# jviquerat/beacon

Hardware: AMD Instinct MI355X
Metric: aggregate env steps/sec, rayleigh-v0 batch=512/GPU 128x64 (higher is better)
Workload: dtype f32

## Files before the change

### beacon_amd/build.py

```python
import fcntl
import glob
import hashlib
import os
import shutil
import subprocess
from concurrent.futures import ThreadPoolExecutor

PKG = os.path.dirname(os.path.abspath(__file__))
CSRC = os.path.join(PKG, "csrc")
INC = os.path.join(os.path.dirname(PKG), "include")
LIB = os.path.join(PKG, "libbeacon_hip.so")
OBJ = os.path.join(PKG, "csrc", "_obj")
ARCH = "gfx950"
FLAGS = ["-O3", "-std=c++17", "-fPIC", "--offload-arch=" + ARCH, "-fvisibility=hidden",
         "-fgpu-rdc" if False else "-fno-gpu-rdc", "-Wall", "-Wno-unused-function",
         "-Wno-unused-variable", "-Wno-unused-but-set-variable"]


FILE_FLAGS = {"ns2d_fast.hip": ["-fno-slp-vectorize", "-ffp-contract=on", "-O2"],
              "ns2d_fast_f64.hip": ["-fno-slp-vectorize", "-ffp-contract=on"],
              "ns2d_fast2.hip": ["-fno-slp-vectorize", "-ffp-contract=on", "-mllvm", "-amdgpu-disable-unclustered-high-rp-reschedule",
                                 "-mllvm", "-amdgpu-sdwa-peephole=0"],
              "ns2d_fast_prm.hip": ["-fno-slp-vectorize", "-ffp-contract=on", "-O2"],
              "ns2d_fast_prm_f64.hip": ["-fno-slp-vectorize", "-ffp-contract=on"],
              "ns2d_fast2_prm.hip": ["-fno-slp-vectorize", "-ffp-contract=on", "-mllvm", "-amdgpu-disable-unclustered-high-rp-reschedule",
                                     "-mllvm", "-amdgpu-sdwa-peephole=0"],
              "env1d_f64.hip": ["-ffp-contract=off"],
              "shkadov_warm_f64.hip": ["-ffp-contract=off"],
              "ode_f64.hip": ["-ffp-contract=off"]}


JIT_FLAGS = ["-fno-slp-vectorize", "-ffp-contract=on"]


def hipcc():
    for c in (os.environ.get("HIPCC"), shutil.which("hipcc"), "/opt/rocm/bin/hipcc"):
        if c and os.path.exists(c):
            return c
    return None


def sources():
    return sorted(glob.glob(os.path.join(CSRC, "*.hip")))


def _deps():
    return (sources() + glob.glob(os.path.join(CSRC, "*.h")) + glob.glob(os.path.join(CSRC, "*.inc")) +
            glob.glob(os.path.join(INC, "*.h")))


def signature():
    h = hashlib.sha256()
    h.update(repr((ARCH, FLAGS, sorted(FILE_FLAGS.items()))).encode())
    for f in sorted(_deps()):
        h.update(os.path.basename(f).encode())
        with open(f, "rb") as fh:
            h.update(fh.read())
    return h.hexdigest()


def stale():
    if not os.path.exists(LIB) or not os.path.exists(LIB + ".sig"):
        return True
    with open(LIB + ".sig") as fh:
        return fh.read().strip() != signature()


def sweep_objdirs():
    if not os.path.isdir(OBJ):
        return
    for d in os.listdir(OBJ):
        if not (d.startswith("p") and d[1:].isdigit()):
            continue
        pid = int(d[1:])
        if pid != os.getpid():
            try:
                os.kill(pid, 0)
                continue
            except ProcessLookupError:
                pass
            except OSError:
                continue
        shutil.rmtree(os.path.join(OBJ, d), ignore_errors=True)


def build_lib(force=False, verbose=False):
    if not force and not stale():
        sweep_objdirs()
        return LIB
    cc = hipcc()
    if cc is None:
        raise RuntimeError("hipcc not found: cannot build libbeacon_hip.so")
    os.makedirs(OBJ, exist_ok=True)
    with open(os.path.join(OBJ, ".lock"), "w") as lock:
        fcntl.flock(lock, fcntl.LOCK_EX)
        try:
            if not force and not stale():
                return LIB
            sig = signature()
            objdir = os.path.join(OBJ, "p%d" % os.getpid())
            os.makedirs(objdir, exist_ok=True)

# ... 29 lines not shown
```

### beacon_amd/csrc/capi.hip

```cpp
#include <math.h>
#include <stdarg.h>
#include <stddef.h>

#include <new>
#include <vector>

#include "env1d.h"
#include "ns2d.h"
#include "ode_env.h"
#include "params.h"
#include "snapshot.h"
#include "episode.h"
#include "shkadov_jets.h"
#include "normalize.h"

static thread_local char g_err[512] = "";

__attribute__((visibility("default"))) void bcn_set_error(const char* fmt, ...) {
  va_list ap;
  va_start(ap, fmt);
  vsnprintf(g_err, sizeof(g_err), fmt, ap);
  va_end(ap);
}

// ... 148 lines not shown
  size_t state_elems() const override { return 4 * (size_t)a.ncell; }
  int get_state(void* buf, int is_device, hipStream_t s) override {
    return copy_planes(buf, fields.p, 4, (size_t)a.ncell * sizeof(real), batch, is_device, s, true);
  }
  int set_state(const void* buf, int is_device, hipStream_t s) override {
    return copy_planes(const_cast<void*>(buf), fields.p, 4, (size_t)a.ncell * sizeof(real), batch, is_device, s, false);
  }
  int set_variant(int v) override { variant = (v == 1 && fast_ok) ? 1 : 0; host.launched = nullptr; return variant; }
  void set_mask(const uint8_t* m) override { a.mask = m; }
  int set_sched(int mode, int grid, int q, int lpt_min_batch) override {
    a.sched_mode = mode; a.sched_grid = grid; a.sched_q_user = q; a.lpt_min_batch = lpt_min_batch;
    return BCN_OK;
  }
  int set_option(const char* name, int value) override {
    if (!strcmp(name, "conv_plan") && value >= 0 && value <= 3) {
      if (value >= 2 && !guard_holds()) { bcn_set_error("conv_plan %d needs a grid with no side below 48 cells (%dx%d): plans 0, 1 only", value, a.nx, a.ny); return BCN_ERR_ARG; }
      a.conv_plan = value;
      return BCN_OK;
    }
    if (!strcmp(name, "plan_overshoot") && value >= 0 && value <= 64) { a.plan_overshoot = value; return BCN_OK; }
    if (!strcmp(name, "verify_conv")) { a.verify_conv = value ? 1 : 0; return BCN_OK; }
    if (!strcmp(name, "spec_start") && value >= 0 && value <= 17) { a.spec_start = value; return BCN_OK; }
    if (!strcmp(name, "transport_iter") && value >= 0 && value <= 64) { a.transport_iter = value; return BCN_OK; }
    if (!strcmp(name, "sched_tail") && value >= 0 && value <= 1024) { host.sched_tail = value; return BCN_OK; }
    if (!strcmp(name, "generic_threads") && (value == 0 || value == 256 || value == 1024)) { host.generic_nt = value; return BCN_OK; }
    if (!strcmp(name, "params_kernel") && (value == 0 || value == 1)) { params_kernel = value; host.launched = nullptr; return BCN_OK; }
    return bcn_env_s::set_option(name, value);
  }
  int get_counters(uint64_t* host, hipStream_t s) override {
    BCN_HIP(hipMemcpyAsync(host, a.cyc, (size_t)batch * 4 * sizeof(uint64_t), hipMemcpyDeviceToHost, s));
    BCN_HIP(hipStreamSynchronize(s));
    return BCN_OK;
  }
  typedef int (*plugin_fn)(const void*, int, void*);
  plugin_fn plugin = nullptr;
  int set_fast_plugin(void* fn, size_t scratch_elems) override {
    plugin_prm = nullptr;
    if (!fn) { plugin = nullptr; fast_ok = ns2d_fast_supported<real>(a); variant = fast_ok ? 1 : 0; return BCN_OK; }
    if (scratch_elems > 0) {
      DeviceGuard g(device);
      fscrbuf.release();
      int rc = fscrbuf.alloc((size_t)batch * scratch_elems * sizeof(real));
      if (rc) return rc;
      BCN_HIP(hipMemset(fscrbuf.p, 0, fscrbuf.bytes));
      a.fscr = static_cast<real*>(fscrbuf.p);
      a.fscr_stride = scratch_elems;
    }
    plugin = reinterpret_cast<plugin_fn>(fn);
    fast_ok = true; variant = 1; host.launched = nullptr;
    return BCN_OK;
  }
  typedef int (*plugin_prm_fn)(const void*, int, void*, const void*);
  plugin_prm_fn plugin_prm = nullptr;
  int set_fast_plugin_params(void* fn) override {
    if (fn && !plugin) { bcn_set_error("bcn_set_fast_plugin_params: the handle has no kernel plugin (bcn_set_fast_plugin comes first)"); return BCN_ERR_ARG; }
    plugin_prm = reinterpret_cast<plugin_prm_fn>(fn);
    host.launched = nullptr;
    return BCN_OK;
  }
  NS2DHost host;
  const real* prm = nullptr;
  int params_kernel = 0;
  void use_params(const void* table) override { prm = static_cast<const real*>(table); host.launched = nullptr; }
  bool prm_fast() const {
    return prm && params_kernel == 1 && variant == 1 && (plugin ? plugin_prm != nullptr : ns2d_fast_supported_prm<real>(a));
  }
  const char* kernel_name() const override {
    if (prm && !prm_fast()) return "ns2d_generic_step";
    return host.launched ? host.launched : (variant == 1 ? "ns2d_fast_step" : "ns2d_generic_step");
  }
  int launch(hipStream_t s) {
    a.host = &host;
    if (prm) {
      if (prm_fast()) {
        const int rc = plugin ? plugin_prm(&a, batch, s, prm) : ns2d_launch_fast_prm<real>(a, batch, s, prm);
        if (rc != BCN_ERR_UNSUPPORTED) return rc;
      }
      return ns2d_launch_generic_prm<real>(a, batch, s, prm);
    }
    if (variant == 1 && plugin) {
      const int rc = plugin(&a, batch, s);
      if (rc != BCN_ERR_UNSUPPORTED) return rc;
      return ns2d_launch_generic<real>(a, batch, s);
    }
    if (variant == 1) return ns2d_launch_fast<real>(a, batch, s);
    return ns2d_launch_generic<real>(a, batch, s);
  }
};

template <typename real>
void ns2d_common(NS2DArgs<real>& a, int nx, int ny, double dx, double dy, double dt, double tol) {
  a.nx = nx; a.ny = ny; a.sx = nx + 2; a.ncell = (nx + 2) * (ny + 2);
  a.dt = (real)dt; a.rdx = (real)(1.0 / dx); a.rdy = (real)(1.0 / dy);
  a.rdx2 = (real)(1.0 / (dx * dx)); a.rdy2 = (real)(1.0 / (dy * dy));
  const double den = dx * dx + dy * dy;
  a.cx = (real)(0.5 * dy * dy / den);
  a.cy = (real)(0.5 * dx * dx / den);
  a.cb = (real)(0.5 * dx * dx * dy * dy / den / dt);
  a.tol = (real)tol;
}

template <typename real>
int make_rayleigh(const bcn_rayleigh_cfg* c, int batch, int dtype, int device, bcn_env_t* out) {
  return make_env<NS2DEnv<real>>(BCN_RAYLEIGH, batch, dtype, device, snap_cfg_hash<bcn_rayleigh_cfg, 12, 9>(c), out, [c](NS2DEnv<real>* e) {
    NS2DArgs<real>& a = e->a;
    ns2d_common(a, c->nx, c->ny, c->dx, c->dy, c->dt, c->tol);
    a.kind = 0; a.ndt_act = c->ndt_act; a.n_act = c->n_act; a.itmax = c->itmax;
    a.n_sgts = c->n_sgts; a.nx_sgts = c->nx_sgts;
    a.nxo = c->nx_obs_pts; a.nyo = c->ny_obs_pts; a.nx_obs = c->nx_obs; a.ny_obs = c->ny_obs;
    a.n_obs_steps = c->n_obs_steps; a.n_obs = 3 * c->n_obs_steps * c->nx_obs_pts * c->ny_obs_pts;
    a.kmom = (real)bcn_rayleigh_kmom(c->pr, c->ra);
    a.ksc = (real)bcn_rayleigh_ksc(c->pr, c->ra);
    e->prm_cfg[0] = c->ra; e->prm_aux[0] = c->pr;
    a.Tc = (real)c->Tc; a.Th = (real)c->Th; a.C = (real)c->C;
    a.rwd_scale = (real)(1.0 / (0.5 * c->dy * c->nx));
    e->n_obs = a.n_obs; e->n_act = c->n_sgts; e->ndt_act = a.ndt_act;
  });
}

template <typename real>
int make_mixing(const bcn_mixing_cfg* c, int batch, int dtype, int device, bcn_env_t* out) {
  return make_env<NS2DEnv<real>>(BCN_MIXING, batch, dtype, device, snap_cfg_hash<bcn_mixing_cfg, 14, 9>(c), out, [c](NS2DEnv<real>* e) {
    NS2DArgs<real>& a = e->a;
    ns2d_common(a, c->nx, c->ny, c->dx, c->dy, c->dt, c->tol);
    a.kind = 1; a.ndt_act = c->ndt_act; a.n_act = c->n_act; a.itmax = c->itmax;
    a.n_sgts = 0; a.nx_sgts = 1;
    a.nxo = c->nx_obs_pts; a.nyo = c->ny_obs_pts; a.nx_obs = c->nx_obs; a.ny_obs = c->ny_obs;
    a.n_obs_steps = c->n_obs_steps; a.n_obs = 3 * c->n_obs_steps * c->nx_obs_pts * c->ny_obs_pts;
    a.i_min = c->i_min; a.i_max = c->i_max; a.j_min = c->j_min; a.j_max = c->j_max;
    a.kmom = (real)bcn_mixing_kmom(c->re);
    a.ksc = (real)bcn_mixing_ksc(c->pe);
    e->prm_cfg[0] = c->re; e->prm_cfg[1] = c->pe; e->prm_aux[0] = c->re; e->prm_aux[1] = c->u_max;
    a.u_max = (real)bcn_mixing_u_max(c->re, c->re, c->u_max); a.ref_c = (real)c->ref_c; a.C0 = (real)c->C0;
    e->n_obs = a.n_obs; e->n_act = 1; e->ndt_act = a.ndt_act;
  });
}

template <typename real>
struct Env1D : bcn_env_s {
  Env1DArgs<real> a{};
  int nfields = 4;
  int nact = 1;
  DevBuf fields, a_last, a_prev, stpbuf, nctrbuf;
  const char* general = "";
  Env1DLaunch last;

  int init() {
    int rc;
    const size_t per = (size_t)batch * a.n * sizeof(real);
    if ((rc = fields.alloc(4 * per))) return rc;
    BCN_HIP(hipMemset(fields.p, 0, 4 * per));
    real* f = static_cast<real*>(fields.p);
    const size_t n = (size_t)batch * a.n;
    a.f0 = f; a.f1 = f + n; a.f2 = f + 2 * n; a.f3 = f + 3 * n;
    if ((rc = a_last.alloc((size_t)batch * nact * sizeof(real)))) return rc;
    if ((rc = a_prev.alloc((size_t)batch * nact * sizeof(real)))) return rc;
    BCN_HIP(hipMemset(a_last.p, 0, a_last.bytes));
    BCN_HIP(hipMemset(a_prev.p, 0, a_prev.bytes));
    a.a_last = static_cast<real*>(a_last.p);
    a.a_prev = static_cast<real*>(a_prev.p);
    if ((rc = stpbuf.alloc((size_t)batch * sizeof(int32_t)))) return rc;
    BCN_HIP(hipMemset(stpbuf.p, 0, stpbuf.bytes));
    stp = a.stp = static_cast<int32_t*>(stpbuf.p);
    if ((rc = nctrbuf.alloc((size_t)batch * sizeof(uint32_t)))) return rc;
    BCN_HIP(hipMemset(nctrbuf.p, 0, nctrbuf.bytes));
    a.nctr = static_cast<uint32_t*>(nctrbuf.p);
// ... 941 lines not shown
```

### beacon_amd/csrc/ns2d.h

```cpp
#pragma once
#include "bcn_common.h"

struct NS2DHost {
  const char* launched = nullptr;
  int sched_tail = 0;
  int generic_nt = 0;
};

template <typename real>
struct NS2DArgs {
  int nx, ny, sx, ncell;
  int ndt_act, n_act, itmax;
  int kind;
  int n_sgts, nx_sgts;
  int nxo, nyo, nx_obs, ny_obs, n_obs_steps, n_obs;
  int i_min, i_max, j_min, j_max;
  real dt, rdx, rdy, rdx2, rdy2;
  real kmom;
  real ksc;
  real cx, cy, cb;
  real tol;
  real Tc, Th, C, u_max, ref_c, C0;
  real rwd_scale;
  real *u, *v, *p, *S, *us, *vs;
  real *g0, *g1, *g2;
  real* obs_hist;
  real* a_last;
  int32_t* ia_last;
  int32_t* stp;
  const real* actions;
  const int32_t* iactions;
  real* actions_norm;
  real* obs_out;
  real* rwd_out;
  uint8_t* done;
  uint8_t* trunc;
  int32_t* status;
  int32_t* sweeps;
  const real* init_fields;
  const uint8_t* mask;
  int work_in_lds;
  int it_begin, it_end;
  int first_chunk, last_chunk;
  const int32_t* order;
  int32_t* order_out;
  int32_t* sweeps_int;
  void* sched_ctl;
  unsigned long long* cyc;
  size_t sched_bytes;
  int sched_q;
  int sched_nbig = 0;
  int conv_plan = 1;
  int plan_overshoot = 0;
  int spec_start = 0;
  int verify_conv = 0;
  int sched_mode = -1;
  int sched_grid = 0, sched_q_user = 0, lpt_min_batch = 0;
  NS2DHost* host;
  real* fscr;
  size_t fscr_stride;
  int transport_iter = 0;
  float slow_l2lc[2] = {0.f, 0.f};
  float slow_cl[2] = {__builtin_inff(), __builtin_inff()};
};

template <typename real> int ns2d_launch_generic(const NS2DArgs<real>& a, int batch, hipStream_t s);
template <typename real> int ns2d_launch_reset(const NS2DArgs<real>& a, int batch, hipStream_t s);
size_t ns2d_generic_lds_bytes(int ncell, size_t esz);
template <typename real> bool ns2d_fast_supported(const NS2DArgs<real>& a);
template <typename real> int ns2d_launch_fast(const NS2DArgs<real>& a, int batch, hipStream_t s);
template <typename real> size_t ns2d_fast_scratch_elems(const NS2DArgs<real>& a);
template <typename real> bool ns2d_fast2_supported(const NS2DArgs<real>& a);
template <typename real> size_t ns2d_fast2_scratch_elems(const NS2DArgs<real>& a);
template <typename real> int ns2d_launch_fast2(const NS2DArgs<real>& a, int batch, hipStream_t s);
```

### beacon_amd/csrc/ns2d_fast.hip

```cpp
#include "ns2d_fast_impl.h"

namespace {

template <typename real>
int fast_config(const NS2DArgs<real>& a) {
  if (a.kind != 0 || a.n_sgts > 64) return 0;
  if (a.nx == 128 && a.ny == 64 && sizeof(real) == 4) return 1;
  if (a.nx == 50 && a.ny == 50) return 2;
  if (a.nx == 128 && a.ny == 64 && sizeof(real) == 8) return 3;
  if (a.nx == 100 && a.ny == 50 && sizeof(real) == 4) return 4;
  if (a.nx == 150 && a.ny == 50 && sizeof(real) == 4) return 5;
  if (a.nx == 200 && a.ny == 50 && sizeof(real) == 4) return 6;
  return 0;
}

}

template <typename real>
bool BCN_PRM_NAME(ns2d_fast_supported)(const NS2DArgs<real>& a) { return fast_config<real>(a) != 0 || BCN_PRM_NAME(ns2d_fast2_supported)<real>(a); }

template <typename real>
int BCN_PRM_NAME(ns2d_launch_fast)(const NS2DArgs<real>& a, int batch, hipStream_t s BCN_PRM_PARAM) {
  if (BCN_PRM_NAME(ns2d_fast2_supported)<real>(a)) return BCN_PRM_NAME(ns2d_launch_fast2)<real>(a, batch, s BCN_PRM_ARG);
  switch (fast_config<real>(a)) {
    case 1:
      if constexpr (std::is_same<real, float>::value) return launch_fast<float, 128, 64, BCN_R128, 0>(a, batch, s BCN_PRM_ARG);
      break;
    case 2: return launch_fast<real, 50, 50, BCN_R50, 0>(a, batch, s BCN_PRM_ARG);
    case 3:
      if constexpr (std::is_same<real, double>::value) return launch_fast<double, 128, 64, BCN_R128D, 0, BCN_GFD>(a, batch, s BCN_PRM_ARG);
      break;
    case 4:
      if constexpr (std::is_same<real, float>::value) return launch_fast<float, 100, 50, 10, 0>(a, batch, s BCN_PRM_ARG);
      break;
    case 5:
      if constexpr (std::is_same<real, float>::value) return launch_fast<float, 150, 50, 15, 0>(a, batch, s BCN_PRM_ARG);
      break;
    case 6:
      if constexpr (std::is_same<real, float>::value) return launch_fast<float, 200, 50, 25, 0>(a, batch, s BCN_PRM_ARG);
      break;
    default: break;
  }
  bcn_set_error("no register-resident kernel for this grid");
  return BCN_ERR_UNSUPPORTED;
}

#ifndef BCN_PRM_KERNELS
template <typename real>
size_t ns2d_fast_scratch_elems(const NS2DArgs<real>& a) {
  if (ns2d_fast2_supported<real>(a)) return ns2d_fast2_scratch_elems<real>(a);
  if (fast_config<real>(a) == 3) return FastGeom<128, 64, BCN_R128D, BCN_GFD>::scratch_elems();
  return 0;
}
#endif
#ifdef BCN_PRM_KERNELS
#ifndef BCN_FAST_TU_F64
template bool ns2d_fast_supported_prm<float>(const NS2DArgs<float>&);
template int ns2d_launch_fast_prm<float>(const NS2DArgs<float>&, int, hipStream_t, const float*);
#else
template bool ns2d_fast_supported_prm<double>(const NS2DArgs<double>&);
template int ns2d_launch_fast_prm<double>(const NS2DArgs<double>&, int, hipStream_t, const double*);
#endif
#elif !defined(BCN_FAST_TU_F64)
template size_t ns2d_fast_scratch_elems<float>(const NS2DArgs<float>&);
template bool ns2d_fast_supported<float>(const NS2DArgs<float>&);
template int ns2d_launch_fast<float>(const NS2DArgs<float>&, int, hipStream_t);
#else
template size_t ns2d_fast_scratch_elems<double>(const NS2DArgs<double>&);
template bool ns2d_fast_supported<double>(const NS2DArgs<double>&);
template int ns2d_launch_fast<double>(const NS2DArgs<double>&, int, hipStream_t);
#endif
```

### beacon_amd/csrc/ns2d_fast_impl.h

```cpp
#pragma once
#include <stdlib.h>

#include <type_traits>

#include "bcn_dpp.h"
#include "ns2d.h"
#include "ns2d_device.h"
#include "ns2d_prm.h"
#include "ns2d_sched.h"


#ifndef BCN_R128
#define BCN_R128 16
#endif
#ifndef BCN_R50
#define BCN_R50 5
#endif
#ifndef BCN_GFD
#define BCN_GFD 2
#endif
#ifndef BCN_PDG
#define BCN_PDG 8
#endif
static_assert(BCN_PDG == 4 || BCN_PDG == 8 || BCN_PDG == 10 || BCN_PDG == 12 || BCN_PDG == 16 || BCN_PDG == 20,
// ... 177 lines not shown
    }                                                                                       \
  }
  constexpr int TA = ((NY - 1 + PD - 1) / PD) * PD;
  constexpr int TB = (NX / PD) * PD;
  if constexpr (TA <= TB) {
    BCN_CHAIN(0, TA, 1)
    if (NY == 64) { BCN_CHAIN(TA, TB, 0) } else { BCN_CHAIN(TA, TB, 1) }
    BCN_CHAIN(TB, NSTEP, 2)
  } else {
    constexpr int TL = ((NY - 1) / PD) * PD, TH = ((NX + PD - 1) / PD) * PD;
    BCN_CHAIN(0, TL, 1)
    BCN_CHAIN(TL, TH, 3)
    BCN_CHAIN(TH, NSTEP, 2)
  }
#undef BCN_CHAIN
}

template <typename real, int NX, int NY, int R0, int RW, int KIND, bool EQ, int GF>
__device__ __forceinline__ void fast_body(const NS2DArgs<real>& A, const int w, const int b, const int it_begin, const int it_end,
                                          const bool first_chunk, const bool last_chunk, char* smem) {
  using G = FastGeom<NX, NY, R0, GF>;
  constexpr int R = RW;
  constexpr int NW = G::NW, NT = G::NT, SY = G::SY, SX = G::SX, SZ = G::SZ, PD = G::PD;
  real* exch = reinterpret_cast<real*>(smem);
  real* errp = exch + G::EXCH;
  real* sact = errp + 128;
  real* red = sact + 64;
  real* gscr = GF ? A.fscr + (size_t)blockIdx.x * A.fscr_stride + G::FRONTG : nullptr;
  real* Ul = GF == 1 ? gscr : GF == 2 ? exch + G::MISCA : exch + G::FRONT;
  real* Vl = Ul + SZ;
  real* Tl = GF == 2 ? gscr : Vl + SZ;

  const int tid = threadIdx.x, lane = tid & 63;
  int j = lane + 1;
  const bool active = lane < NY;
  constexpr int RL = G::RL;
  constexpr bool DEADC = GF == 2 && RW == R0 && RL != R0;
  static_assert(!(DEADC && G::XC == 4), "dead columns exist only in the single-sweep exchange paths (XC == 2, GF == 2)");
  const bool lastw = DEADC && w == NW - 1;
#define LIVE(k) (!DEADC || (k) < RL || !lastw)
  const int i0 = w * R0 + 1;
  const size_t off = (size_t)b * A.ncell;
  real* __restrict__ gu = A.u + off;
  real* __restrict__ gv = A.v + off;
  real* __restrict__ gp = A.p + off;
  real* __restrict__ gS = A.S + off;
  constexpr int XC = G::XC, XL = XC - 1;
  auto exl = [&](int buf, int wave, int which) -> real& { return exch[((buf * NW + wave) * XC + which) * 64 + lane]; };

  for (int c = tid; c < SX * SY; c += NT) {
    const int jj = c / SX, ii = c - jj * SX;
    Ul[ii * SY + jj] = gu[c];
    Vl[ii * SY + jj] = gv[c];
    Tl[ii * SY + jj] = gS[c];
  }
  for (int c = SX * SY + tid; c < SZ; c += NT) { Ul[c] = 0; Vl[c] = 0; Tl[c] = 0; }
  if (tid < 128) errp[tid] = 0;
  real p[R];
#pragma unroll
  for (int k = 0; k < R; k++) p[k] = (active && LIVE(k)) ? gp[j * SX + i0 + k] : real(0);

  if (!first_chunk) {
    if (tid < A.n_sgts) sact[tid] = A.a_last[(size_t)b * A.n_sgts + tid];
  } else {
    const int n = A.n_sgts;
    const real* src = A.actions ? A.actions + (size_t)b * n : A.a_last + (size_t)b * n;
    real mean = 0;
    for (int k = 0; k < n; k++) mean += src[k];
    mean /= (real)n;
    real m = 1;
    for (int k = 0; k < n; k++) {
      real t = bcn_abs(src[k] - mean) / A.C;
      m = t > m ? t : m;
    }
    real mine = (tid < n) ? (src[tid] - mean) / m : real(0);
    __syncthreads();
    if (tid < n) {
      sact[tid] = mine;
      A.a_last[(size_t)b * n + tid] = mine;
      if (A.actions_norm) A.actions_norm[(size_t)b * n + tid] = mine;
    }
  }
  __syncthreads();

  const real dt = A.dt, rdx = A.rdx, rdy = A.rdy, rdx2 = A.rdx2, rdy2 = A.rdy2;
  const real cx = A.cx, cy = A.cy;
  const real wl = active ? real(1) + (j == 1 ? 1 : 0) + ((j == NY && KIND == 0) ? 1 : 0) : real(0);
  const real fW = (active && w == 0) ? real(1) : real(0);
  const real fE = (active && w == NW - 1) ? real(1) : real(0);
  const real cW = wl + fW, cE = lastw ? real(0) : wl + fE;
  const real fEl = lastw ? fE : real(0);
  const real cBy = cy * (real)((lane == 0 ? 1 : 0) + ((lane == NY - 1 && KIND == 0) ? 1 : 0));
  const real actf = active ? real(1) : real(0);

  int status = 0;
  int xb = 0;
#ifdef BCN_STAMP
  const unsigned long long kt0 = __builtin_amdgcn_s_memtime(), kr0 = __builtin_amdgcn_s_memrealtime();
  unsigned long long seg[7] = {0, 0, 0, 0, 0, 0, 0};
  unsigned long long tl = kt0;
#define BCN_PH(x) { __builtin_amdgcn_sched_barrier(0); const unsigned long long t__ = __builtin_amdgcn_s_memtime(); seg[x] += t__ - tl; tl = t__; __builtin_amdgcn_sched_barrier(0); }
#else
#define BCN_PH(x)
#endif
  if (!first_chunk) status = A.status[b];
  const unsigned long long cyc_u0 = __builtin_amdgcn_s_memtime();
  unsigned long long cyc_j = 0;
  real* const prev_sweeps = red + 20;
  constexpr bool SPEC = std::is_same<real, float>::value;
#if !defined(BCN_STAMP) && !defined(BCN_DBG_NCHK)
  if (tid == 0) prev_sweeps[0] = (it_begin > 0 && A.sweeps) ? (real)A.sweeps[(size_t)b * A.ndt_act + it_begin - 1] : real(0);
#else
  if (tid == 0) prev_sweeps[0] = 0;
#endif
  if (tid == 0) { prev_sweeps[1] = 0; prev_sweeps[2] = 0; prev_sweeps[3] = 0; }
  real* const slow_k = red + 24;
  if (tid == 0) {
    slow_k[0] = 0; slow_k[5] = 0;
    slow_k[1] = (real)A.slow_l2lc[0]; slow_k[2] = (real)A.slow_cl[0];
    slow_k[3] = (real)A.slow_l2lc[1]; slow_k[4] = (real)A.slow_cl[1];
  }

  constexpr bool OFFLOAD = G::template offload<real>();
  real* const P0 = exch + G::base_elems();
  real* const US0 = P0 + R0 * 64;
  real* const VX0 = US0 + R0 * 64;
  auto pred = [&](const int i, real uc, real uE_, real uW_, real uN_, real uS_, real uSE_, real vc, real vE_, real vW_, real vN_,
                  real vS_, real vNW_, real pc, real pW, real pS, real& us_out, real& vx_out) {
    {
      real uE = real(0.5) * (uE_ + uc), uW = real(0.5) * (uc + uW_);
      real uN2 = real(0.5) * (uN_ + uc), uS2 = real(0.5) * (uc + uS_);
      real vN2 = real(0.5) * (vN_ + vNW_), vS2 = real(0.5) * (vc + vW_);
      real conv = (uE * uE - uW * uW) * rdx + (uN2 * vN2 - uS2 * vS2) * rdy;
      real diff = ((uE_ - 2 * uc + uW_) * rdx2 + (uN_ - 2 * uc + uS_) * rdy2) * A.kmom;
      real pres = (pc - pW) * rdx;
      us_out = (i >= 2 && (!DEADC || i <= NX) && active) ? uc + dt * (diff - conv - pres) : real(0);
    }
    {
      real vE = real(0.5) * (vE_ + vc), vW = real(0.5) * (vc + vW_);
      real uE = real(0.5) * (uE_ + uSE_), uW = real(0.5) * (uc + uS_);
      real vN2 = real(0.5) * (vN_ + vc), vS2 = real(0.5) * (vc + vS_);
      real conv = (uE * vE - uW * vW) * rdx + (vN2 * vN2 - vS2 * vS2) * rdy;
      real diff = ((vE_ - 2 * vc + vW_) * rdx2 + (vN_ - 2 * vc + vS_) * rdy2) * A.kmom;
      real pres = (pc - pS) * rdy;
      vx_out = diff - conv - pres;
    }
  };
  auto bc_uv = [&]() {
    for (int jj = 1 + tid; jj <= NY; jj += NT) {
      Ul[1 * SY + jj] = 0;
      Ul[(NX + 1) * SY + jj] = 0;
      if (jj >= 2) {
        Vl[0 * SY + jj] = -Vl[1 * SY + jj];
        Vl[(NX + 1) * SY + jj] = -Vl[NX * SY + jj];
      }
    }
    for (int ii = 1 + tid; ii <= NX + 1; ii += NT) {
      const bool wall = (ii == 1) || (ii == NX + 1);
      const real utop = wall ? real(0) : Ul[ii * SY + NY];
      const real ubot = wall ? real(0) : Ul[ii * SY + 1];
      Ul[ii * SY + NY + 1] = -utop;
      Ul[ii * SY + 0] = -ubot;
      if (ii <= NX) {
        Vl[ii * SY + NY + 1] = 0;
        Vl[ii * SY + 1] = 0;
      }
    }
  };
  auto publish_p = [&]() {
    exl(xb, w, 1) = p[R - 1];
    if (OFFLOAD && w == 0) {
#pragma unroll
      for (int k = 0; k < R; k++) P0[k * 64 + lane] = p[k];
    }
  };

  bc_uv();
  publish_p();
  __syncthreads();

  real us[R], vs[R];
  for (int it = it_begin;; it++) {
    asm volatile("" : "+v"(j));
    const bool have_chain = it > it_begin;
    const bool have_pred = it < it_end && status == 0;
    real vx[R];
    const bool pred_own = have_pred && (w != 0 || !have_chain);
    if (w == 0 && have_chain) {
#ifndef BCN_CHAIN_PRIO
#define BCN_CHAIN_PRIO 3
#endif
      __builtin_amdgcn_s_setprio(BCN_CHAIN_PRIO);
// ... 35 lines not shown
      if (have_pred && have_chain && w != 0) {
        constexpr int CH0 = 4, NCH0 = (R0 + CH0 - 1) / CH0;
        static_assert(NCH0 <= NW - 1, "one chunk of strip 0 per helper wave");
        const int c = (NW == 8) ? (w < 4 ? w - 1 : (w == 4 ? 6 : w - 2)) : w - 1;
        if (c < NCH0) {
          const int kc = c * CH0;
          real ur[CH0 + 2], uS[CH0 + 1], uN[CH0], vr[CH0 + 2], vN[CH0 + 1], vS[CH0], pp[CH0 + 1];
          const int ic = 1 + kc;
#pragma unroll
          for (int k = 0; k < CH0 + 2; k++) { ur[k] = Ul[(ic - 1 + k) * SY + j]; vr[k] = Vl[(ic - 1 + k) * SY + j]; }
#pragma unroll
          for (int k = 0; k < CH0 + 1; k++) { uS[k] = Ul[(ic + k) * SY + j - 1]; vN[k] = Vl[(ic - 1 + k) * SY + j + 1]; }
#pragma unroll
          for (int k = 0; k < CH0; k++) { uN[k] = Ul[(ic + k) * SY + j + 1]; vS[k] = Vl[(ic + k) * SY + j - 1]; }
#pragma unroll
          for (int k = 0; k <= CH0; k++) {
            const int kk = kc + k - 1;
            const int kq = kk < 0 ? 0 : (kk < R0 ? kk : R0 - 1);
            const real pv = P0[kq * 64 + lane];
            pp[k] = (kk >= 0 && kk < R0) ? pv : real(0);
          }
#pragma unroll
          for (int k = 0; k < CH0; k++) {
            const int kk = kc + k;
            const real pc = pp[k + 1];
            const real pS = from_below(pc, pc);
            real uo, xo;
            pred(ic + k, ur[k + 1], ur[k + 2], ur[k], uN[k], uS[k], uS[k + 1], vr[k + 1], vr[k + 2], vr[k], vN[k + 1], vS[k], vN[k],
                 pc, pp[k], pS, uo, xo);
            if (kk < R0) {
              US0[kk * 64 + lane] = uo;
              VX0[kk * 64 + lane] = xo;
            }
          }
        }
      }
    }
    if (w != 0) { BCN_PH(6) }
    if (have_pred) xb ^= 1;
    if (have_pred && w != 0) exl(xb, w, 0) = us[0];
    __syncthreads();
    BCN_PH(5)
    if (!have_pred) break;
    asm volatile("" : "+v"(j));
    if (w == 0 && have_chain) {
      if constexpr (OFFLOAD) {
#pragma unroll
        for (int k = 0; k < R; k++) { us[k] = US0[k * 64 + lane]; vx[k] = VX0[k * 64 + lane]; }
      } else {
        BCN_OWN_PRED
      }
    }
#undef BCN_OWN_PRED
    constexpr bool TREG = GF == 2 && KIND == 0;
    real Tr[TREG ? R : 1];
    if constexpr (TREG) {
#pragma unroll
      for (int k = 0; k < R; k++) Tr[k] = Tl[(i0 + k) * SY + j];
      if (active) {
        if (w == 0) Tl[0 * SY + j] = Tr[0];
        if (w == NW - 1) Tl[(NX + 1) * SY + j] = Tr[(DEADC ? RL : R) - 1];
      }
      {
        real gt = 0, gb = 0;
#pragma unroll
        for (int k = 0; k < R; k++) {
          const real tt = read_lane(Tr[k], NY - 1), tb = read_lane(Tr[k], 0);
          gt = (lane == k) ? 2 * A.Tc - tt : gt;
          gb = (lane == k) ? tb : gb;
        }
        const int ii = i0 + (lane < R ? lane : 0);
        const int sg = (ii - 1) / A.nx_sgts;
        const real sa = sact[sg < A.n_sgts ? sg : 0];
        if (lane < (lastw ? RL : R)) {
          Tl[ii * SY + NY + 1] = gt;
          if (sg < A.n_sgts) Tl[ii * SY + 0] = 2 * (A.Th + sa) - gb;
        }
      }
    } else {
    for (int jj = 1 + tid; jj <= NY; jj += NT) {
      Tl[0 * SY + jj] = Tl[1 * SY + jj];
      Tl[(NX + 1) * SY + jj] = Tl[NX * SY + jj];
    }
    for (int ii = 1 + tid; ii <= NX; ii += NT) {
      Tl[ii * SY + NY + 1] = 2 * A.Tc - Tl[ii * SY + NY];
      const int k = (ii - 1) / A.nx_sgts;
      if (k < A.n_sgts) Tl[ii * SY + 0] = 2 * (A.Th + sact[k]) - Tl[ii * SY + 1];
    }
    }
#pragma unroll
    for (int k = 0; k < R; k++) {
      const real buoy = (KIND == 0) ? (TREG ? Tr[TREG ? k : 0] : Tl[(i0 + k) * SY + j]) : real(0);
      vs[k] = (j >= 2 && active && LIVE(k)) ? Vl[(i0 + k) * SY + j] + dt * (vx[k] + buoy) : real(0);
    }
    BCN_PH(0)

    real nb[R];
    {
      const real usE = (w < NW - 1) ? exl(xb, w + 1, 0) : real(0);
      xb ^= 1;
#pragma unroll
      for (int k = 0; k < R; k++) {
        const real ue = (k < R - 1) ? us[k < R - 1 ? k + 1 : 0] : usE;
        const real vn = from_above(real(0), vs[k]);
        nb[k] = (active && LIVE(k)) ? -A.cb * ((ue - us[k]) * rdx + (vn - vs[k]) * rdy) : real(0);
      }
    }
    const int wm = (w > 0) ? w - 1 : 0, wp = (w < NW - 1) ? w + 1 : NW - 1;
    real nbW = 0, nbE = 0;
    if constexpr (XC == 4) {
      exl(xb, w, 0) = nb[0];
      exl(xb, w, 3) = nb[R - 1];
      real a1p = 0;
#pragma unroll
      for (int k = 0; k < R; k++) a1p += nb[k] * nb[k];
      const real a1w = wave_sum_lane63<real>(a1p);
      if (lane == 63) exch[((xb * NW + w) * XC + 1) * 64] = a1w;
      __syncthreads();
      nbW = exl(xb, wm, 3);
      nbE = exl(xb, wp, 0);
      const real a1q = (lane < NW) ? exch[((xb * NW + (lane < NW ? lane : 0)) * XC + 1) * 64] : real(0);
      const real a1 = read_lane(row16_sum<real>(a1q), 15);
      if (tid == 0) slow_k[0] = (real)(0.5f * __log2f(3.f * (float)a1 / (float)A.tol));
      xb ^= 1;
    } else if (A.conv_plan == 3) {
      real a1p = 0;
#pragma unroll
      for (int k = 0; k < R; k++) a1p += nb[k] * nb[k];
      const real a1w = wave_sum_lane63<real>(a1p);
      if (lane == 63) errp[(xb ^ 1) * 64 + w] = a1w;
      __syncthreads();
      const real a1 = read_lane(row16_sum<real>(errp[(xb ^ 1) * 64 + (lane & 15)]), 15);
      if (tid == 0) slow_k[0] = (real)(0.5f * __log2f(3.f * (float)a1 / (float)A.tol));
    }

    BCN_PH(1)
    const unsigned long long cyc_j0 = __builtin_amdgcn_s_memtime();
    auto cell = [&](real c, real e, real wv, real nbk) -> real {
      const real q = cBy * c + nbk;
      real ph;
      if constexpr (EQ && std::is_same<real, float>::value) {
        ph = jacobi_cell_eq(c, e, wv, nbk, cx, cBy);
      } else if (EQ) {
        real sum = e + wv;
        sum = add_above_below(sum, c);
        ph = cx * sum + q;
      } else {
        const real ns = dpp<0x130, 0xf, 0xf, true>(real(0), c) + dpp<0x138, 0xf, 0xf, true>(real(0), c);
        ph = cx * (e + wv) + (cy * ns + q);
      }
      if (NY < 64) ph *= actf;
      return ph;
    };
    real hW = 0, hE = 0;
    real hW1r, hW2r, hE1r, hE2r;
    int itp;
    real phA[R], phB[R];
    bool finalB;
    const real tolL0 = (A.conv_plan == 3) ? A.tol * real(BCN_CONV_GUARD) : A.tol;
    const float l2tol_u = __log2f((float)A.tol * 1.02f), l2tol_w = __log2f((float)tolL0 * 1.003f);
    constexpr int JMAX = 256;
#ifdef BCN_DBG_NCHK
    int nchk = 0;
#define BCN_NCHK_INC nchk++;
#else
#define BCN_NCHK_INC
#endif
#ifdef BCN_STAMP
    const unsigned long long st0 = __builtin_amdgcn_s_memtime();
#endif
    for (;;) {
    hW1r = 0; hW2r = 0; hE1r = 0; hE2r = 0;
    itp = 0;
#pragma unroll
    for (int k = 0; k < R; k++) phA[k] = 0;
    finalB = false;
    real tolL = tolL0;
    int k_prev = -1;
    float l2u_prev = 0, l2w_prev = 0;
    int skip_left = 0;
    const int plan = (A.conv_plan == 3) ? (__builtin_amdgcn_readfirstlane((int)prev_sweeps[1]) != 0 ? 1 : 2) : A.conv_plan;
#define BCN_CELLS(SRC, DST)                                                                  \
      _Pragma("unroll") for (int k = 1; k < R - 1; k++) DST[k] = cell(SRC[k], SRC[k + 1], SRC[k - 1], nb[k]); \
         \
      __builtin_amdgcn_sched_barrier(0);                                                     \
      hW = (w > 0) ? hW1r : SRC[0];                                                          \
      hE = (w < NW - 1) ? hE1r : SRC[R - 1];                                                 \
      const real p0 = cell(SRC[0], SRC[1], hW, nb[0]);                                       \
      const real pl = cell(SRC[R - 1], hE, SRC[R - 2], nb[R - 1]);                           \
      DST[0] = p0;                                                                           \
      DST[R - 1] = pl;                                                                       \
       \
      if constexpr (DEADC) DST[DEADC ? RL : 0] = lastw ? DST[DEADC ? RL - 1 : 0] : DST[DEADC ? RL : 0]; \
      BCN_PUBLISH(DST)
#define BCN_PUBLISH(DST)                                                                     \
      exl(xb, w, 0) = DST[0];                                                                \
      exl(xb, w, XL) = DST[R - 1];                                                           \
      if constexpr (XC == 4) { exl(xb, w, 1) = DST[1]; exl(xb, w, 2) = DST[R - 2]; }
#define BCN_HALO_READS                                                                       \
      hW1r = exl(xb, wm, XL);                                                                \
      hE1r = exl(xb, wp, 0);                                                                 \
      if constexpr (XC == 4) { hW2r = exl(xb, wm, 2); hE2r = exl(xb, wp, 1); }               \
      xb ^= 1;
#define BCN_SWEEP_END                                                                        \
// ... 126 lines not shown
      real acc2 = 0;                                                                         \
      _Pragma("unroll") for (int k = 1; k < R - 1; k++) { const real d = X[k] - Y[k]; acc2 += d * d; } \
      const real d20 = X[0] - Y[0], d2l = X[R - 1] - Y[R - 1];                               \
      const real part2 = wl * acc2 + cW * (d20 * d20) + cE * (d2l * d2l);                    \
      const real t1_63 = wave_sum_lane63<real>(part1), t2_63 = wave_sum_lane63<real>(part2); \
      if (lane == 63) { errp[xb * 64 + w] = t1_63; errp[xb * 64 + 16 + w] = t2_63; }         \
      if (plan == 1) {    \
        const real u1_63 = wave_sum_lane63<real>(upart1);                                    \
        const real u2_63 = wave_sum_lane63<real>(acc2 + d20 * d20 + d2l * d2l);              \
        if (lane == 63) { errp[xb * 64 + 32 + w] = u1_63; errp[xb * 64 + 48 + w] = u2_63; }  \
      }                                                                                      \
      __syncthreads();                                                                       \
      itp += 2;                                                                              \
      const real epart = errp[xb * 64 + lane];                                               \
      BCN_HALO_READS                                                                         \
      const real esum = row16_sum<real>(epart);                                              \
      const real err1 = read_lane(esum, 15), err2 = read_lane(esum, 31);                     \
       \
      const bool ov1 = itp - 1 > A.itmax, ov2 = itp > A.itmax;                               \
      const bool pass1 = ov1 || !(err1 > A.tol), pass2 = ov2 || !(err2 > A.tol);             \
       \
      const bool amb = SPEC && skip_left == -2 && plan == 1 && !(read_lane(esum, 47) > A.tol * real(1.02)); \
       \
      const bool unv = plan >= 2 && !A.verify_conv && itp0 > 0 && k_prev != itp0 && !(err1 > tolL); \
      if (pass1 || pass2 || amb || unv) {                                                    \
        const bool ovf = ov1 || (ov2 && (err1 > A.tol));                                     \
        if (ovf) status |= BCN_ST_ITMAX;                                                     \
        if (!ovf && skip_left > (pass1 ? 0 : 1)) status |= BCN_ST_PLAN;    \
        if (SPEC) skip_left = (skip_left == -2 && !ovf) ? -1 : 0;                            \
        finalB = pass1;                                                                      \
        itp -= pass1 ? 1 : 0;                                                                \
         \
        hW1r = pass1 ? yw : hW1r;                                                            \
         \
        late_stop = unv && !ovf;                                                             \
        break;                                                                               \
      }                                                                                      \
      if (SPEC) skip_left = skip_left < 0 ? 0 : skip_left;                                   \
      n = 0;                                                                                 \
      if (skip_left > 0) {                                                                   \
        skip_left = skip_left > 2 ? skip_left - 2 : 0;                                       \
      } else if (plan > 0) {                       \
        int j = 0;                                                                           \
        if (plan == 1) {                                                                     \
          const float l2u1 = __log2f((float)read_lane(esum, 47)), l2u2 = __log2f((float)read_lane(esum, 63)); \
          const float room_u = l2u2 - l2tol_u, rho_u = l2u2 - l2u1;                          \
          if (room_u > 0.f) j = (rho_u < 0.f) ? (int)fminf(room_u / -rho_u, (float)JMAX) : JMAX; \
        } else {                                                                             \
          const float l2w1 = __log2f((float)err1), l2w2 = __log2f((float)err2);              \
          float l2tl = l2tol_w;                                                              \
          if (A.conv_plan == 3) {    \
            const float e0 = (float)slow_k[0], fi = (float)itp;                              \
            const float t0 = 1.f + 2.f * exp2f(e0 + fi * (float)slow_k[1]), t1 = 1.f + 2.f * exp2f(e0 + fi * (float)slow_k[3]); \
            const float g = fminf(fminf((float)slow_k[2] * t0 * t0, (float)slow_k[4] * t1 * t1) * 1.001f, (float)BCN_CONV_GUARD); \
            tolL = A.tol * (real)g;                                                          \
            l2tl = __log2f((float)tolL * 1.003f);                                            \
          }                                                                                  \
          const float room_w = l2w2 - l2tl, rho_w = l2w2 - l2w1;                             \
          if (SPEC && tid == 0) slow_k[5] = (real)-rho_w;    \
          int jw = 0;                                                                        \
          if (room_w > 0.f) jw = (rho_w < 0.f) ? (int)fminf(room_w / -rho_w, (float)JMAX) : JMAX; \
          j = jw - 1 - (jw >> 4) + A.plan_overshoot;                                         \
          j = j > 0 ? j : 0;                                                                 \
        }                                                                                    \
        j = __builtin_amdgcn_readfirstlane(j) & ~1;                                          \
        k_prev = itp;                                                                        \
        if (A.verify_conv) skip_left = j; else n = j;                                        \
      }                                                                                      \
    }
    constexpr bool PAIRS = XC == 4;
    bool late_stop = false;
    if constexpr (SPEC && XC == 4) {
      if (A.spec_start > 0 && plan > 1 && !A.verify_conv) {
        const int prev = __builtin_amdgcn_readfirstlane((int)prev_sweeps[0]);
        int n0 = (prev * (A.spec_start <= 16 ? A.spec_start : 6)) >> 3;
        if (A.spec_start == 17 && plan == 2 && A.conv_plan == 3) {
          const float rp = (float)slow_k[5];
          if (rp > 0.f) n0 = ((prev * 15) >> 4) - (int)fminf(ceilf(BCN_OPEN_ZONE_L2 / rp), 4096.f);
        }
        n0 = __builtin_amdgcn_readfirstlane(n0) & ~1;
        if (n0 > A.itmax) n0 = A.itmax & ~1;
        if (prev >= 16 && n0 > 0) {
          skip_left = -2;
          for (; n0 > 0; n0 -= 2) BCN_FAST2X(phA, phB)
        }
      }
    }
    if constexpr (PAIRS) {
      for (;;) {
        int n;
        BCN_CHECK2X(phA, phB)
        if (n > A.itmax - itp) n = (A.itmax - itp > 0 ? A.itmax - itp : 0) & ~1;
        for (; n > 0; n -= 2) BCN_FAST2X(phA, phB)
      }
    } else {
    for (;;) {
      int n;
      BCN_CHECK(phA, phB, true)
      if (n == 0) {
        BCN_CHECK(phB, phA, false)
        n &= ~1;
      } else {
        BCN_FAST(phB, phA)
        n = (n - 1) & ~1;
      }
      if (SPEC && XC != 4 && itp == 2 && A.spec_start > 0 && plan > 0 && !A.verify_conv) {
        const int prev = __builtin_amdgcn_readfirstlane((int)prev_sweeps[0]);
        const int ns = ((prev * (A.spec_start <= 16 ? A.spec_start : 6)) >> 3) - 2;
        if (prev >= 16 && ns > n) { n = ns & ~1; skip_left = -2; }
      }
      if (n > A.itmax - itp) n = (A.itmax - itp > 0 ? A.itmax - itp : 0) & ~1;
      if constexpr (XC == 4) {
        for (; n > 0; n -= 2) BCN_FAST2X(phA, phB)
      } else {
        for (; n > 0; n -= 2) {
          BCN_FAST(phA, phB)
          BCN_FAST(phB, phA)
        }
      }
    }
    late_stop = itp >= 2 && k_prev != itp - 2;
    }
#undef BCN_CHECK2X
#undef BCN_CHECK
#undef BCN_FAST2X
#undef BCN_HALO_READS
#undef BCN_PUBLISH
#undef BCN_FAST
#undef BCN_SWEEP_END
#undef BCN_CELLS
    {
      const bool toofar = SPEC && skip_left == -1;
      const bool late = plan >= 2 && !toofar && late_stop && !(status & BCN_ST_ITMAX);
      if (late && tid == 0) prev_sweeps[2] += 1;
      if (!(toofar || (late && A.conv_plan == 3))) {
        if (tid == 0) { prev_sweeps[0] = SPEC ? (real)itp : real(0); prev_sweeps[1] = 0; }
        break;
      }
      if (tid == 0) { prev_sweeps[0] = 0; prev_sweeps[1] = toofar ? real(0) : real(1); prev_sweeps[3] += 1; }
      __syncthreads();
    }
    }
    if (finalB) {
#pragma unroll
      for (int k = 0; k < R; k++) phA[k] = phB[k];
    }
    hW = hW1r;
#ifdef BCN_STAMP
    {
      const unsigned long long st1 = __builtin_amdgcn_s_memtime();
      const int cps = (int)((st1 - st0) / (unsigned long long)(itp > 0 ? itp : 1));
      if (A.sweeps && tid == 0) A.sweeps[(size_t)b * A.ndt_act + it] = itp | (cps << 16);
    }
#elif defined(BCN_DBG_NCHK)
    if (A.sweeps && tid == 0) A.sweeps[(size_t)b * A.ndt_act + it] = itp | (nchk << 16);
#else
    if (A.sweeps && tid == 0) A.sweeps[(size_t)b * A.ndt_act + it] = itp;
#endif

    cyc_j += __builtin_amdgcn_s_memtime() - cyc_j0;
    asm volatile("" : "+v"(j));
    BCN_PH(2)
#pragma unroll
    for (int k = 0; k < R; k++) {
      const int i = i0 + k;
      const real ph = phA[k];
// ... 202 lines not shown
```

### beacon_amd/csrc/ns2d_fast_prm.hip

```cpp
#define BCN_PRM_KERNELS 1
#include "params.h"
#include "ns2d_fast.hip"
```

### beacon_amd/jit.py

```python
import ctypes as C
import fcntl
import hashlib
import os
import subprocess
import warnings

from . import build as _build

class JitWarning(UserWarning):
    """Every warning of this module: a plugin that could not be built / loaded / checked, or that failed its self-check.
    tests/conftest.py turns the category into an error, so a refused plugin is a red test, not a line in a log."""


JIT_DIR = os.path.join(_build.PKG, "_jit")
JIT_SRC = os.path.join(_build.CSRC, "jit", "ns2d_jit.hip")
LDS_BYTES = 160 * 1024
_LOADED = {}


def _up16(x):
    return (x + 15) // 16 * 16


def _lds_rows1(nx, ny, nw, esz, gf, r=0):
# ... 173 lines not shown

    v, text = _verdict_on_disk(p, tag)
    if v is not None:
        return settle(v, text)
    lock = None
    try:
        lock = open(p.path + ".vlock", "w")
        fcntl.flock(lock, fcntl.LOCK_EX)
    except OSError:
        lock = None
    try:
        v, text = _verdict_on_disk(p, tag)
        if v is not None:
            return settle(v, text)
        CHECKING = True
        try:
            ok, rep = compare_with_generic(make_env, kind, f64, params=params)
        except Exception as e:
            warnings.warn("beacon_amd.jit: the self-check of %s could not run (%s: %s); the generic kernel stays selected for this env"
                          % (os.path.basename(p.path), type(e).__name__, e), JitWarning)
            return
        finally:
            CHECKING = False
        p.verified, p.report = bool(ok), rep
        try:
            with open(p.path + (".ok" if ok else ".bad"), "w") as fh:
                fh.write("%s\n%s\n" % (tag, rep))
            try:
                os.remove(p.path + (".bad" if ok else ".ok"))
            except FileNotFoundError:
                pass
            if lock is not None:
                os.remove(p.path + ".vlock")
        except OSError:
            pass
    finally:
        if lock is not None:
            fcntl.flock(lock, fcntl.LOCK_UN)
            lock.close()
    if not ok:
        warnings.warn("beacon_amd.jit: the register-resident kernel %s DISAGREES with the generic kernel on its self-check (%s); "
                      "it is not used: the generic kernel stays selected" % (os.path.basename(p.path), rep), JitWarning)


def selftest(device="cuda:0", verbose=False):
    from . import vec as V
    cases = [("rayleigh 128x64", 0, dict(L=2.56, H=1.28), ("f32", "f64")), ("rayleigh 50x50", 0, dict(), ("f32", "f64")),
             ("rayleigh 100x50", 0, dict(L=2.0), ("f32",)), ("rayleigh 150x50", 0, dict(L=3.0), ("f32",)),
             ("rayleigh 200x50", 0, dict(L=4.0), ("f32",)), ("rayleigh 100x100", 0, dict(L=2.0, H=2.0), ("f32",)),
             ("mixing 100x100", 1, dict(), ("f32", "f64"))]
    out = {}
    for name, kind, kw, dts in cases:
        for dt in dts:
            if kind == 0:
                mk = lambda B, dt=dt, kw=kw: V.VecRayleigh(B, device, dt, None, **kw)
            else:
                mk = lambda B, dt=dt, kw=kw: V.VecMixing(B, device, dt, **kw)
            ok, rep = compare_with_generic(mk, kind, dt == "f64")
            out["%s %s" % (name, dt)] = (ok, rep)
            if verbose:
                print("%-24s %s  %s" % (name + " " + dt, "ok " if ok else "BAD", rep), flush=True)
    return out


def _signature(defs):
    h = hashlib.sha256()
    h.update(repr((_build.ARCH, _build.FLAGS, _build.JIT_FLAGS, sorted(defs.items()))).encode())
    for f in sorted([JIT_SRC] + [os.path.join(_build.CSRC, n) for n in os.listdir(_build.CSRC) if n.endswith(".h")] +
                    [os.path.join(_build.INC, n) for n in os.listdir(_build.INC) if n.endswith(".h")]):
        h.update(os.path.basename(f).encode())
        with open(f, "rb") as fh:
            h.update(fh.read())
    return h.hexdigest()[:12]


def build_plugin(nx, ny, f64, kind, verbose=False, extra_defs=None):
    m = choose(nx, ny, f64, kind)
    if m is None or os.environ.get("BEACON_JIT", "1") == "0":
        return None
    defs = {"BCN_JIT_ROWS": m["rows"], "BCN_JIT_REAL": "double" if f64 else "float", "BCN_JIT_NX": nx, "BCN_JIT_NY": ny,
            "BCN_JIT_R": m["R"], "BCN_JIT_KIND": kind, "BCN_JIT_GF": m["gf"]}
    if m["rows"] == 4:
        defs["BCN_JIT_RPL"] = m["rpl"]
    for d in os.environ.get("BEACON_JIT_DEFS", "").split():
        defs[d.partition("=")[0]] = d.partition("=")[2] or "1"
    defs.update(extra_defs or {})
    name = "ns2d_%dx%d_%s_k%d_r%d_%s.so" % (nx, ny, "f64" if f64 else "f32", kind, m["R"], _signature(defs))
    path = os.path.join(JIT_DIR, name)
    if os.path.exists(path):
        return path
    cc = _build.hipcc()
    if cc is None or os.environ.get("BEACON_NO_BUILD") == "1":
        return None
    tmp = "%s.tmp%d" % (path, os.getpid())
    try:
        os.makedirs(JIT_DIR, exist_ok=True)
        with open(path + ".lock", "w") as lock:
            fcntl.flock(lock, fcntl.LOCK_EX)
            try:
                if os.path.exists(path):
                    return path
                cmd = ([cc] + _build.FLAGS + _build.JIT_FLAGS +
                       ["-D%s=%s" % kv for kv in sorted(defs.items())] + ["-I", _build.INC, "-shared", JIT_SRC, "-o", tmp])
                if verbose:
                    print(" ".join(cmd), flush=True)
                subprocess.check_call(cmd)
                os.replace(tmp, path)
            finally:
                fcntl.flock(lock, fcntl.LOCK_UN)
    except (OSError, subprocess.CalledProcessError) as e:
        warnings.warn("beacon_amd.jit: no register-resident kernel for %dx%d (%s); the generic kernel stays selected"
                      % (nx, ny, e), JitWarning)
        try:
            os.remove(tmp)
        except OSError:
            pass
        return None
    return path


class Plugin(object):
    def __init__(self, path):
        self.path = path
        self.lib = C.CDLL(path)
        self.lib.bcn_jit_scratch_elems.restype = C.c_size_t
        self.lib.bcn_jit_lds_bytes.restype = C.c_size_t
        self.fn = C.cast(self.lib.bcn_jit_launch, C.c_void_p)
        self.fn_prm = C.cast(self.lib.bcn_jit_launch_prm, C.c_void_p) if hasattr(self.lib, "bcn_jit_launch_prm") else None
        self.scratch = int(self.lib.bcn_jit_scratch_elems())
        self.lds = int(self.lib.bcn_jit_lds_bytes())
        self.verified = None
        self.report = ""


def plugin_for(nx, ny, f64, kind, extra_defs=None):
    key = (nx, ny, bool(f64), kind, tuple(sorted((extra_defs or {}).items())))
    if key not in _LOADED:
        path = build_plugin(nx, ny, f64, kind, extra_defs=extra_defs)
        try:
            p = Plugin(path) if path else None
        except (OSError, AttributeError) as e:
            warnings.warn("beacon_amd.jit: cannot load %s (%s); the generic kernel stays selected" % (path, e), JitWarning)
            p = None
        if p is not None and p.lds > LDS_BYTES:
            p = None
        _LOADED[key] = p
    return _LOADED[key]


TEST_GRIDS = [(75, 50, False, 0), (75, 50, True, 0), (53, 50, False, 0), (110, 64, False, 0), (110, 64, True, 0),
              (50, 70, False, 0), (60, 120, False, 0), (100, 110, False, 1), (150, 50, True, 0), (110, 65, False, 0),
              (100, 105, False, 1), (50, 70, True, 0), (50, 150, False, 0), (50, 150, True, 0), (64, 200, False, 0),
              (100, 200, False, 1), (50, 145, False, 0), (50, 149, True, 0), (100, 130, False, 1),
              (300, 50, False, 0), (200, 100, False, 1), (53, 150, False, 0), (106, 200, False, 1),
              (50, 75, True, 0), (57, 107, True, 0), (100, 105, True, 1), (50, 75, False, 0),
              (52, 50, True, 0), (125, 55, True, 0)]


def fuzz_grids(seed=5):
    import numpy as np
    rng = np.random.default_rng(seed)
    quota = {(1, False): 4, (1, True): 3, (2, False): 4, (2, True): 3, (4, False): 6, (4, True): 2}
    out = []
    while any(quota.values()):
        kind = int(rng.integers(0, 2))
        f64 = bool(rng.integers(0, 2))
# ... 154 lines not shown
```

Before: 29640.

## Add opening-phase variant with bottom-BC table and warm-started speculative Poisson sweeps

New measurement: 29820 (median of 6 runs). No clear change (+0.6%).

```diff
diff --git a/beacon_amd/build.py b/beacon_amd/build.py
--- a/beacon_amd/build.py
+++ b/beacon_amd/build.py
@@ -18,6 +18,7 @@
 
 
 FILE_FLAGS = {"ns2d_fast.hip": ["-fno-slp-vectorize", "-ffp-contract=on", "-O2"],
+              "ns2d_fast_open.hip": ["-fno-slp-vectorize", "-ffp-contract=on", "-O2"],
               "ns2d_fast_f64.hip": ["-fno-slp-vectorize", "-ffp-contract=on"],
               "ns2d_fast2.hip": ["-fno-slp-vectorize", "-ffp-contract=on", "-mllvm", "-amdgpu-disable-unclustered-high-rp-reschedule",
                                  "-mllvm", "-amdgpu-sdwa-peephole=0"],
diff --git a/beacon_amd/csrc/capi.hip b/beacon_amd/csrc/capi.hip
--- a/beacon_amd/csrc/capi.hip
+++ b/beacon_amd/csrc/capi.hip
@@ -254,6 +254,9 @@
       const int rc = plugin(&a, batch, s);
       if (rc != BCN_ERR_UNSUPPORTED) return rc;
       return ns2d_launch_generic<real>(a, batch, s);
+    }
+    if constexpr (std::is_same<real, float>::value) {
+      if (variant == 1) return ns2d_launch_fast_open<float>(a, batch, s);
     }
     if (variant == 1) return ns2d_launch_fast<real>(a, batch, s);
     return ns2d_launch_generic<real>(a, batch, s);
diff --git a/beacon_amd/csrc/ns2d.h b/beacon_amd/csrc/ns2d.h
--- a/beacon_amd/csrc/ns2d.h
+++ b/beacon_amd/csrc/ns2d.h
@@ -69,6 +69,7 @@
 size_t ns2d_generic_lds_bytes(int ncell, size_t esz);
 template <typename real> bool ns2d_fast_supported(const NS2DArgs<real>& a);
 template <typename real> int ns2d_launch_fast(const NS2DArgs<real>& a, int batch, hipStream_t s);
+template <typename real> int ns2d_launch_fast_open(const NS2DArgs<real>& a, int batch, hipStream_t s);
 template <typename real> size_t ns2d_fast_scratch_elems(const NS2DArgs<real>& a);
 template <typename real> bool ns2d_fast2_supported(const NS2DArgs<real>& a);
 template <typename real> size_t ns2d_fast2_scratch_elems(const NS2DArgs<real>& a);
diff --git a/beacon_amd/csrc/ns2d_fast.hip b/beacon_amd/csrc/ns2d_fast.hip
--- a/beacon_amd/csrc/ns2d_fast.hip
+++ b/beacon_amd/csrc/ns2d_fast.hip
@@ -1,4 +1,10 @@
 #include "ns2d_fast_impl.h"
+
+#ifdef BCN_OPEN_UNIT
+#define BCN_FAST_NAME(f) f##_open
+#else
+#define BCN_FAST_NAME(f) BCN_PRM_NAME(f)
+#endif
 
 namespace {
 
@@ -17,10 +23,10 @@
 }
 
 template <typename real>
-bool BCN_PRM_NAME(ns2d_fast_supported)(const NS2DArgs<real>& a) { return fast_config<real>(a) != 0 || BCN_PRM_NAME(ns2d_fast2_supported)<real>(a); }
+bool BCN_FAST_NAME(ns2d_fast_supported)(const NS2DArgs<real>& a) { return fast_config<real>(a) != 0 || BCN_PRM_NAME(ns2d_fast2_supported)<real>(a); }
 
 template <typename real>
-int BCN_PRM_NAME(ns2d_launch_fast)(const NS2DArgs<real>& a, int batch, hipStream_t s BCN_PRM_PARAM) {
+int BCN_FAST_NAME(ns2d_launch_fast)(const NS2DArgs<real>& a, int batch, hipStream_t s BCN_PRM_PARAM) {
   if (BCN_PRM_NAME(ns2d_fast2_supported)<real>(a)) return BCN_PRM_NAME(ns2d_launch_fast2)<real>(a, batch, s BCN_PRM_ARG);
   switch (fast_config<real>(a)) {
     case 1:
@@ -45,7 +51,7 @@
   return BCN_ERR_UNSUPPORTED;
 }
 
-#ifndef BCN_PRM_KERNELS
+#if !defined(BCN_PRM_KERNELS) && !defined(BCN_OPEN_UNIT)
 template <typename real>
 size_t ns2d_fast_scratch_elems(const NS2DArgs<real>& a) {
   if (ns2d_fast2_supported<real>(a)) return ns2d_fast2_scratch_elems<real>(a);
@@ -53,7 +59,9 @@
   return 0;
 }
 #endif
-#ifdef BCN_PRM_KERNELS
+#if defined(BCN_OPEN_UNIT)
+template int ns2d_launch_fast_open<float>(const NS2DArgs<float>&, int, hipStream_t);
+#elif defined(BCN_PRM_KERNELS)
 #ifndef BCN_FAST_TU_F64
 template bool ns2d_fast_supported_prm<float>(const NS2DArgs<float>&);
 template int ns2d_launch_fast_prm<float>(const NS2DArgs<float>&, int, hipStream_t, const float*);
diff --git a/beacon_amd/csrc/ns2d_fast_impl.h b/beacon_amd/csrc/ns2d_fast_impl.h
--- a/beacon_amd/csrc/ns2d_fast_impl.h
+++ b/beacon_amd/csrc/ns2d_fast_impl.h
@@ -283,6 +283,19 @@
     }
   }
   __syncthreads();
+#if defined(BCN_OPENING) && !defined(BCN_NO_TBOT_TABLE)
+  constexpr bool TBOT = GF == 0 && std::is_same<real, float>::value;
+#else
+  constexpr bool TBOT = false;
+#endif
+  static_assert(!TBOT || G::BACK >= NX + 1, "the bottom-value table fits the back pad");
+  real* const tbot = exch + G::FRONT + 3 * SZ + G::BACK - (NX + 1);
+  if constexpr (TBOT) {
+    for (int ii = 1 + tid; ii <= NX; ii += NT) {
+      const int k = (ii - 1) / A.nx_sgts;
+      tbot[ii] = 2 * (A.Th + sact[k < A.n_sgts ? k : 0]);
+    }
+  }
 
   const real dt = A.dt, rdx = A.rdx, rdy = A.rdy, rdx2 = A.rdx2, rdy2 = A.rdy2;
   const real cx = A.cx, cy = A.cy;
@@ -309,6 +322,11 @@
   unsigned long long cyc_j = 0;
   real* const prev_sweeps = red + 20;
   constexpr bool SPEC = std::is_same<real, float>::value;
+#if defined(BCN_OPENING) && !defined(BCN_NO_PHI1)
+  constexpr bool PHI1 = SPEC && G::XC == 4;
+#else
+  constexpr bool PHI1 = false;
+#endif
 #if !defined(BCN_STAMP) && !defined(BCN_DBG_NCHK)
   if (tid == 0) prev_sweeps[0] = (it_begin > 0 && A.sweeps) ? (real)A.sweeps[(size_t)b * A.ndt_act + it_begin - 1] : real(0);
 #else
@@ -510,10 +528,18 @@
       Tl[0 * SY + jj] = Tl[1 * SY + jj];
       Tl[(NX + 1) * SY + jj] = Tl[NX * SY + jj];
     }
+    if constexpr (TBOT) {
+      const int ncov = A.n_sgts * A.nx_sgts;
+      for (int ii = 1 + tid; ii <= NX; ii += NT) {
+        Tl[ii * SY + NY + 1] = 2 * A.Tc - Tl[ii * SY + NY];
+        if (ii <= ncov) Tl[ii * SY + 0] = tbot[ii] - Tl[ii * SY + 1];
+      }
+    } else {
     for (int ii = 1 + tid; ii <= NX; ii += NT) {
       Tl[ii * SY + NY + 1] = 2 * A.Tc - Tl[ii * SY + NY];
       const int k = (ii - 1) / A.nx_sgts;
       if (k < A.n_sgts) Tl[ii * SY + 0] = 2 * (A.Th + sact[k]) - Tl[ii * SY + 1];
+    }
     }
     }
 #pragma unroll
@@ -539,15 +565,19 @@
     if constexpr (XC == 4) {
       exl(xb, w, 0) = nb[0];
       exl(xb, w, 3) = nb[R - 1];
+      if constexpr (PHI1) { exl(xb, w, 1) = nb[1]; exl(xb, w, 2) = nb[R - 2]; }
+      auto a1s = [&](int q) -> real& {
+        if constexpr (PHI1) return errp[xb * 64 + q]; else return exch[((xb * NW + q) * XC + 1) * 64];
+      };
       real a1p = 0;
 #pragma unroll
       for (int k = 0; k < R; k++) a1p += nb[k] * nb[k];
       const real a1w = wave_sum_lane63<real>(a1p);
-      if (lane == 63) exch[((xb * NW + w) * XC + 1) * 64] = a1w;
+      if (lane == 63) a1s(w) = a1w;
       __syncthreads();
       nbW = exl(xb, wm, 3);
       nbE = exl(xb, wp, 0);
-      const real a1q = (lane < NW) ? exch[((xb * NW + (lane < NW ? lane : 0)) * XC + 1) * 64] : real(0);
+      const real a1q = (lane < NW) ? a1s(lane < NW ? lane : 0) : real(0);
       const real a1 = read_lane(row16_sum<real>(a1q), 15);
       if (tid == 0) slow_k[0] = (real)(0.5f * __log2f(3.f * (float)a1 / (float)A.tol));
       xb ^= 1;
@@ -840,6 +870,16 @@
         if (n0 > A.itmax) n0 = A.itmax & ~1;
         if (prev >= 16 && n0 > 0) {
           skip_left = -2;
+          if constexpr (PHI1) {
+            hW2r = exl(xb ^ 1, wm, 2) + real(0);
+            hE2r = exl(xb ^ 1, wp, 1) + real(0);
+            hW1r = nbW + real(0);
+            hE1r = nbE + real(0);
+#pragma unroll
+            for (int k = 0; k < R; k++) phA[k] = nb[k] + real(0);
+            itp = 1;
+            n0 -= 2;
+          }
           for (; n0 > 0; n0 -= 2) BCN_FAST2X(phA, phB)
         }
       }
diff --git a/beacon_amd/csrc/ns2d_fast_open.hip b/beacon_amd/csrc/ns2d_fast_open.hip
--- /dev/null
+++ b/beacon_amd/csrc/ns2d_fast_open.hip
@@ -0,0 +1,3 @@
+#define BCN_OPENING 1
+#define BCN_OPEN_UNIT 1
+#include "ns2d_fast.hip"
diff --git a/beacon_amd/csrc/ns2d_fast_prm.hip b/beacon_amd/csrc/ns2d_fast_prm.hip
--- a/beacon_amd/csrc/ns2d_fast_prm.hip
+++ b/beacon_amd/csrc/ns2d_fast_prm.hip
@@ -1,3 +1,4 @@
 #define BCN_PRM_KERNELS 1
+#define BCN_OPENING 1
 #include "params.h"
 #include "ns2d_fast.hip"
diff --git a/beacon_amd/jit.py b/beacon_amd/jit.py
--- a/beacon_amd/jit.py
+++ b/beacon_amd/jit.py
@@ -279,6 +279,8 @@
             "BCN_JIT_R": m["R"], "BCN_JIT_KIND": kind, "BCN_JIT_GF": m["gf"]}
     if m["rows"] == 4:
         defs["BCN_JIT_RPL"] = m["rpl"]
+    if m["rows"] == 1 and not f64:
+        defs["BCN_OPENING"] = 1
     for d in os.environ.get("BEACON_JIT_DEFS", "").split():
         defs[d.partition("=")[0]] = d.partition("=")[2] or "1"
     defs.update(extra_defs or {})
```
